# srndpty/kobato-eyes

Hardware: AMD Instinct MI355X
Metric: images/s (pHash + all-pairs Hamming scan + cluster membership) (higher is better)
Workload: dtype u8 luma, int32 taps (i8 matrix cores), f64 DCT, 1-bit Hamming products (fp4 matrix cores, exact)

## Files before the change

kobato-eyes_amd/csrc/ke_hash.hip:

```cpp
#include <cstdlib>

#include "ke_internal.h"
#include "dct_table.h"
#include "ke_hash_select.h"
#include "ke_resample_plan.h"

namespace {

constexpr int kPrecisionBits = 22;

__device__ __forceinline__ int clip8_fixed(int acc) {
    int v = acc >> kPrecisionBits;
    return v < 0 ? 0 : (v > 255 ? 255 : v);
}

__device__ __forceinline__ int luma_of(const uint8_t *p, int ch) {
    if (ch == 1) return p[0];
    return (int)((19595u * p[0] + 38470u * p[1] + 7471u * p[2] + 0x8000u) >> 16);
}

template <int AXIS>
__global__ __launch_bounds__(256) void ke_resample_pass(const uint8_t *__restrict__ src,
                                                         const uint64_t *__restrict__ offsets, uint64_t stride,
                                                         int ch, int w, int h, const int32_t *__restrict__ bounds,
// ... 159 lines not shown
    tile32_coeffs<false>(s_tile, s_T, s_cf[0], tid);
    tile32_coeffs<true>(s_tile, s_T, s_cf[1], tid);
    for (int k = wv; k < 8; k += 4) {
        const float *base = s_cf[k >> 2];
        auto coef = [&](int i) {
            const bool neg = ((k & 1) && (i & 1)) != ((k & 2) && ((i >> 3) & 1));
            return neg ? -base[i] : base[i];
        };
        float r[8];
#pragma unroll
        for (int j = 0; j < 8; ++j) r[j] = coef(1 + j);
#pragma unroll
        for (int i = 8; i < 56; i += 8)
#pragma unroll
            for (int j = 0; j < 8; ++j) r[j] = r[j] + coef(1 + i + j);
        float res = ((r[0] + r[1]) + (r[2] + r[3])) + ((r[4] + r[5]) + (r[6] + r[7]));
#pragma unroll
        for (int i = 56; i < 63; ++i) res = res + coef(1 + i);
        const float mean = res / 63.0f;
        const unsigned long long m = __ballot(coef(lane) > mean);
        if (lane == 0) turned[slot * 8 + k] = __brevll(m);
    }
}

__device__ __forceinline__ uint32_t luma4_biased(uint32_t d0, uint32_t d1, uint32_t d2) {
    constexpr uint32_t CHI = 0x001D964Cu, CLO = 0x002F468Bu, START = 0x8000u - 0x800000u;
    const uint32_t p0 = d0;
    const uint32_t p1 = __builtin_amdgcn_alignbyte(d1, d0, 3);
    const uint32_t p2 = __builtin_amdgcn_alignbyte(d2, d1, 2);
    const uint32_t s0 = (__builtin_amdgcn_udot4(p0, CHI, 0u, false) << 8) + __builtin_amdgcn_udot4(p0, CLO, START, false);
    const uint32_t s1 = (__builtin_amdgcn_udot4(p1, CHI, 0u, false) << 8) + __builtin_amdgcn_udot4(p1, CLO, START, false);
    const uint32_t s2 = (__builtin_amdgcn_udot4(p2, CHI, 0u, false) << 8) + __builtin_amdgcn_udot4(p2, CLO, START, false);
    const uint32_t s3 = (__builtin_amdgcn_udot4(d2, CHI << 8, 0u, false) << 8) + __builtin_amdgcn_udot4(d2, CLO << 8, START, false);
    const uint32_t lo = __builtin_amdgcn_perm(s1, s0, 0x0C0C0602u);
    const uint32_t hi = __builtin_amdgcn_perm(s3, s2, 0x06020C0Cu);
    return lo | hi;
}

template <int C>
__device__ __forceinline__ uint32_t luma4_generic(const uint32_t *d) {
    if (C == 3) return luma4_biased(d[0], d[1], d[2]);
    if (C == 1) return d[0] ^ 0x80808080u;
    constexpr uint32_t CHI = 0x001D964Cu, CLO = 0x002F468Bu, START = 0x8000u - 0x800000u;
    uint32_t s[4];
#pragma unroll
    for (int k = 0; k < 4; ++k)
        s[k] = (__builtin_amdgcn_udot4(d[k], CHI, 0u, false) << 8) + __builtin_amdgcn_udot4(d[k], CLO, START, false);
    return __builtin_amdgcn_perm(s[1], s[0], 0x0C0C0602u) | __builtin_amdgcn_perm(s[3], s[2], 0x06020C0Cu);
}

__device__ __forceinline__ int combine_planes(int d0, int d1, int d2, int bias) {
    return (int)((uint32_t)d0 + ((uint32_t)d1 << 8) + ((uint32_t)d2 << 16) + (uint32_t)bias);
}

struct KeFusedArgs {
    const uint8_t *pixels;
    const uint64_t *offsets;
    uint64_t stride;
    const int64_t *out_idx;
    int h;
    const int32_t *mx_frag;
    int mx_base0, mx_base1;
    const int32_t *h_bias;
    const int32_t *v_packed, *v_start, *v_bias;
    int ndwv;
    int qw, qw_inv, lp;
    int w, row_bytes;
    int lt_half;
    int lt_bytes;
    int hp;
    uint64_t *phash;
    float *margin;
    uint8_t *tile32_out;
    const int32_t *mxd_frag, *hd_bias;
    const int32_t *vd_cpacked, *vd_cstart, *vd_bias;
    int ndwcv;
    int hpd;
    int x_off;
    int bands, band_rows;
    uint8_t *hs, *hsd;
    int hs_hp, hsd_hp;
    uint64_t *dhash;
    uint8_t *tile98_out;
};

template <int C>
__device__ __forceinline__ void patch_last_quad(const uint8_t *image_last_row, int w, uint8_t *lds_row) {
    for (int x = w & ~3; x < w; ++x) lds_row[x] = (uint8_t)(luma_of(image_last_row + (size_t)x * C, C) ^ 0x80);
}

__device__ __forceinline__ void band_writeout(const uint8_t *HT, int hp, int ncols, int rows, uint8_t *dst, int dst_hp, int tid,
                                              int nthreads) {
    const int wpc = (rows + 3) / 4;
    for (int e = tid; e < ncols * wpc; e += nthreads) {
        const int col = e / wpc, k = e % wpc;
        *reinterpret_cast<uint32_t *>(dst + (size_t)col * dst_hp + 4 * k) = *reinterpret_cast<const uint32_t *>(HT + col * hp + 4 * k);
    }
}

template <int NDWD>
__device__ __forceinline__ void fused_tail(const KeFusedArgs &a, uint8_t *Lt, const uint8_t *HT, const uint8_t *HTd,
                                           const int tid, const int64_t img) {
    uint8_t *T32 = Lt;
    double *Td = reinterpret_cast<double *>(Lt + 1024);
    float *cf = reinterpret_cast<float *>(Lt + 1024 + 2048);
    {
        const int yy = tid & 31, og = tid >> 5;
        const int rotv = (yy >> 4) & 1;
        const int vst = a.v_start[yy];
        const int ndwv = a.ndwv;
        int acc[4][3];
#pragma unroll
        for (int m = 0; m < 4; ++m) acc[m][0] = acc[m][1] = acc[m][2] = 0;
        for (int j = 0; j < ndwv; j += 2) {
            const int jj = j ^ (2 * rotv);
            const int32_t *cp = a.v_packed + ((size_t)yy * ndwv + jj) * 3;
            const int c00 = cp[0], c01 = cp[1], c02 = cp[2], c10 = cp[3], c11 = cp[4], c12 = cp[5];
#pragma unroll
            for (int m = 0; m < 4; ++m) {
                const uint2 v = *reinterpret_cast<const uint2 *>(
                    __builtin_assume_aligned(HT + (size_t)(og + 8 * m) * a.hp + vst + 4 * jj, 8));
                acc[m][0] = __builtin_amdgcn_sdot4((int)v.x, c00, acc[m][0], false);
                acc[m][1] = __builtin_amdgcn_sdot4((int)v.x, c01, acc[m][1], false);
                acc[m][2] = __builtin_amdgcn_sdot4((int)v.x, c02, acc[m][2], false);
                acc[m][0] = __builtin_amdgcn_sdot4((int)v.y, c10, acc[m][0], false);
                acc[m][1] = __builtin_amdgcn_sdot4((int)v.y, c11, acc[m][1], false);
                acc[m][2] = __builtin_amdgcn_sdot4((int)v.y, c12, acc[m][2], false);
            }
        }
        const int vbias = a.v_bias[yy];
#pragma unroll
        for (int m = 0; m < 4; ++m)
            T32[yy * 32 + og + 8 * m] = (uint8_t)clip8_fixed(combine_planes(acc[m][0], acc[m][1], acc[m][2], vbias));
    }
    __syncthreads();
    if (a.tile32_out)
        reinterpret_cast<uint32_t *>(a.tile32_out + (size_t)img * 1024)[tid] = reinterpret_cast<const uint32_t *>(T32)[tid];
    const int64_t slot = a.out_idx ? a.out_idx[img] : img;
    const uint64_t hv = tile32_to_phash(T32, Td, cf, tid, (a.margin && a.phash) ? a.margin + slot : nullptr);
    if (tid == 0 && a.phash) a.phash[slot] = hv;
    if (NDWD > 0) {
        __syncthreads();
        int *part = reinterpret_cast<int *>(Lt);
        uint8_t *T98 = Lt + 1024;
        if (tid < 216) {
            const int out = tid / 3, chunk = tid % 3;
            const int yy = out / 9, oc = out % 9;
            const int vc = yy * 3 + chunk;
            const int vst = a.vd_cstart[vc];
            const int nd = a.ndwcv;
            int d0 = 0, d1 = 0, d2 = 0;
            for (int j = 0; j < nd; j += 2) {
                const int32_t *cp = a.vd_cpacked + ((size_t)vc * nd + j) * 3;
                const uint2 v = *reinterpret_cast<const uint2 *>(__builtin_assume_aligned(HTd + (size_t)oc * a.hpd + vst + 4 * j, 8));
                d0 = __builtin_amdgcn_sdot4((int)v.x, cp[0], d0, false);
                d1 = __builtin_amdgcn_sdot4((int)v.x, cp[1], d1, false);
                d2 = __builtin_amdgcn_sdot4((int)v.x, cp[2], d2, false);
                d0 = __builtin_amdgcn_sdot4((int)v.y, cp[3], d0, false);
                d1 = __builtin_amdgcn_sdot4((int)v.y, cp[4], d1, false);
                d2 = __builtin_amdgcn_sdot4((int)v.y, cp[5], d2, false);
            }
            part[tid] = combine_planes(d0, d1, d2, 0);
        }
        __syncthreads();
        if (tid < 72) {
            const int yy = tid / 9;
            const uint32_t sum = (uint32_t)part[3 * tid] + (uint32_t)part[3 * tid + 1] + (uint32_t)part[3 * tid + 2] + (uint32_t)a.vd_bias[yy];
            T98[tid] = (uint8_t)clip8_fixed((int)sum);
        }
        __syncthreads();
        if (a.tile98_out && tid < 72) a.tile98_out[(size_t)img * 72 + tid] = T98[tid];
        if (tid < 64) {
            const int r = tid >> 3, c = tid & 7;
            const unsigned long long m = __ballot(T98[r * 9 + c + 1] > T98[r * 9 + c]);
            if (tid == 0 && a.dhash) a.dhash[a.out_idx ? a.out_idx[img] : img] = __brevll(m);
        }
    }
}

int upload_dct_tables(ke_ctx *ctx) {
    if (ctx->dct_tables_ready) return KE_OK;
    KE_HIP(ctx, hipMemcpyToSymbol(HIP_SYMBOL(c_C32), KE_C32, sizeof(KE_C32)));
    KE_HIP(ctx, hipMemcpyToSymbol(HIP_SYMBOL(c_C16), KE_C16, sizeof(KE_C16)));
    KE_HIP(ctx, hipMemcpyToSymbol(HIP_SYMBOL(c_C8), KE_C8, sizeof(KE_C8)));
    ctx->dct_tables_ready = true;
    return KE_OK;
}

constexpr int kRTM = kKeTileRowsMx;
typedef int ke_v4i __attribute__((ext_vector_type(4)));

template <int W64, int KS, bool DH, bool GEN, int C, bool UNAL>
__global__ __launch_bounds__(256, 2) void ke_phash_fused_mx(const KeFusedArgs a) {
    static_assert(!UNAL || GEN, "rows that are not a multiple of 4 pixels need the run-time row length");
    constexpr uint32_t QB = 4u * C;
    constexpr int W = 64 * W64;
    constexpr int QPT = kRTM * (W / 4) / 256;
    const int QW = GEN ? a.qw : W / 4;
    const int QUADS_PER_TILE = kRTM * QW;
    const int LP = GEN ? a.lp : W + 16;
    constexpr int KD = (W64 + 1) / 2;
    extern __shared__ __attribute__((aligned(16))) uint8_t smem[];
    uint8_t *Lt = smem;
    uint8_t *HT = smem + a.lt_bytes;
    uint8_t *HTd = HT + 32 * a.hp;
    uint8_t *X = smem + a.x_off;
    const int tid = threadIdx.x;
    const int lane = tid & 63, wv = tid >> 6;
    const int64_t img = a.bands ? blockIdx.x / a.bands : blockIdx.x;
    const int y_begin = a.bands ? (int)(blockIdx.x % a.bands) * a.band_rows : 0;
    const uint32_t row_bytes = UNAL ? (uint32_t)a.row_bytes : (uint32_t)QW * QB;
    const uint8_t *src = a.pixels + (a.offsets ? a.offsets[img] : (uint64_t)img * a.stride) + (size_t)y_begin * row_bytes;
    const int h = a.bands ? min(a.band_rows, a.h - y_begin) : a.h;
    const uint32_t image_bytes = (uint32_t)(a.h - y_begin) * row_bytes;

    const int mt = wv >> 1, jt = wv & 1;
    ke_v4i bf[KS][3];
#pragma unroll
    for (int s = 0; s < KS; ++s)
#pragma unroll
        for (int p = 0; p < 3; ++p)
            bf[s][p] = reinterpret_cast<const ke_v4i *>(a.mx_frag)[((jt * KS + s) * 3 + p) * 64 + lane];
    constexpr int KDR = DH ? KD : 1;
    ke_v4i bd[KDR][3];
    int dbias = 0;
    if (DH) {
#pragma unroll
        for (int d = 0; d < KDR; ++d)
#pragma unroll
            for (int p = 0; p < 3; ++p)
                bd[d][p] = reinterpret_cast<const ke_v4i *>(a.mxd_frag)[((jt * KD + d) * 3 + p) * 64 + lane];
        dbias = a.hd_bias[(lane & 15) < 9 ? (lane & 15) : 8];
    }
    const int ocol = 16 * jt + (lane & 15);
    const int hbias = a.h_bias[ocol];
    const int a_off = (16 * mt + (lane & 15)) * LP + (jt ? a.mx_base1 : a.mx_base0) + 16 * (lane >> 4);
    const int d_off = (16 * mt + (lane & 15)) * LP + 64 * KD * jt + 16 * (lane >> 4);
    uint8_t *ht_dst = HT + (size_t)ocol * a.hp + 16 * mt + 4 * (lane >> 4);
    uint8_t *htd_dst = HTd + (size_t)(lane & 15) * a.hpd + 16 * mt + 4 * (lane >> 4);
    ke_v4i *x_slot = reinterpret_cast<ke_v4i *>(X + mt * 1024 + lane * 16);

    uint32_t raw[QPT][C];
    auto load_tile = [&](int t) {
// ... 46 lines not shown
        }
        if (DH) {
            const uint8_t *dp = cur + d_off;
#pragma unroll
            for (int d = 0; d < KDR; ++d) {
                const ke_v4i av = *reinterpret_cast<const ke_v4i *>(__builtin_assume_aligned(dp + 64 * d, 16));
#pragma unroll
                for (int p = 0; p < 3; ++p) dacc[p] = __builtin_amdgcn_mfma_i32_16x16x64_i8(av, bd[d][p], dacc[p], 0, 0, 0);
            }
        }
        *reinterpret_cast<uint32_t *>(ht_dst + t * kRTM) = pack_rows(acc[0], acc[1], acc[2], hbias);
        ke_v4i part;
#pragma unroll
        for (int i = 0; i < 4; ++i) part[i] = combine_planes(dacc[0][i], dacc[1][i], dacc[2][i], 0);
        return part;
    };
    ke_v4i carry = {0, 0, 0, 0};
    auto finish_dhash = [&](int t) {
        const ke_v4i other = x_slot[(t & 1) * 128];
        const ke_v4i zero = {0, 0, 0, 0};
        const ke_v4i sum = carry + other;
        const uint32_t packed = pack_rows(sum, zero, zero, dbias);
        if ((lane & 15) < 9) *reinterpret_cast<uint32_t *>(htd_dst + t * kRTM) = packed;
    };
    auto hpass = [&](int t, const uint8_t *cur) {
        if (!DH) {
            products(t, cur);
        } else if (jt) {
            x_slot[(t & 1) * 128] = products(t, cur);
        } else {
            if (t > 0) finish_dhash(t - 1);
            carry = products(t, cur);
        }
    };

    const int ntiles = (h + kRTM - 1) / kRTM;
    load_tile(0);
    store_luma(Lt);
    __syncthreads();
    for (int t = 0; t + 1 < ntiles; ++t) {
        load_tile(t + 1);
        __builtin_amdgcn_sched_barrier(0);
        hpass(t, Lt + (t & 1) * a.lt_half);
        __builtin_amdgcn_sched_barrier(0);
        store_luma(Lt + ((t + 1) & 1) * a.lt_half);
        __syncthreads();
    }
    if (UNAL) {
        if (tid == 0 && y_begin + h == a.h)
            patch_last_quad<C>(src + (size_t)(h - 1) * row_bytes, a.w, Lt + ((ntiles - 1) & 1) * a.lt_half + ((h - 1) - (ntiles - 1) * kRTM) * LP);
        __syncthreads();
    }
    hpass(ntiles - 1, Lt + ((ntiles - 1) & 1) * a.lt_half);
    __syncthreads();
    if (DH) {
        if (!jt) finish_dhash(ntiles - 1);
        __syncthreads();
    }
    if (a.bands) {
        band_writeout(HT, a.hp, 32, h, a.hs + (size_t)img * 32 * a.hs_hp + y_begin, a.hs_hp, tid, 256);
        if (DH) band_writeout(HTd, a.hpd, 9, h, a.hsd + (size_t)img * 9 * a.hsd_hp + y_begin, a.hsd_hp, tid, 256);
        return;
    }
    fused_tail<(DH ? 1 : 0)>(a, Lt, HT, HTd, tid, img);
}

constexpr int kRTW = kKeTileRowsWide;

template <int KSH, int QPT, bool DH, int KDW, int C, bool UNAL>
__global__ __launch_bounds__(512, 1) void ke_phash_fused_wide(const KeFusedArgs a) {
    constexpr uint32_t QB = 4u * C;
    extern __shared__ __attribute__((aligned(16))) uint8_t smem[];
    uint8_t *Lt = smem;
    uint8_t *HT = smem + a.lt_bytes;
    uint8_t *HTd = HT + 32 * a.hp;
    uint8_t *X = smem + a.x_off;
    const int tid = threadIdx.x;
    const int lane = tid & 63, wv = tid >> 6;
    const int jt = wv & 1, kh = wv >> 1;
    const int64_t img = a.bands ? blockIdx.x / a.bands : blockIdx.x;
    const int y_begin = a.bands ? (int)(blockIdx.x % a.bands) * a.band_rows : 0;
    const int QW = a.qw, LP = a.lp;
    const uint32_t row_bytes = UNAL ? (uint32_t)a.row_bytes : (uint32_t)QW * QB;
    const uint8_t *src = a.pixels + (a.offsets ? a.offsets[img] : (uint64_t)img * a.stride) + (size_t)y_begin * row_bytes;
    const int h = a.bands ? min(a.band_rows, a.h - y_begin) : a.h;
    const int quads_per_tile = kRTW * QW;
    const uint32_t image_bytes = (uint32_t)(a.h - y_begin) * row_bytes;

    ke_v4i bf[KSH][3];
#pragma unroll
    for (int s = 0; s < KSH; ++s)
#pragma unroll
        for (int p = 0; p < 3; ++p)
            bf[s][p] = reinterpret_cast<const ke_v4i *>(a.mx_frag)[((jt * 4 * KSH + kh * KSH + s) * 3 + p) * 64 + lane];
    const int ocol = 16 * jt + (lane & 15);
    const int hbias = a.h_bias[ocol];
    const int a_off = (lane & 15) * LP + (jt ? a.mx_base1 : a.mx_base0) + 64 * KSH * kh + 16 * (lane >> 4);
    uint8_t *ht_dst = HT + (size_t)ocol * a.hp + 4 * (lane >> 4);
    ke_v4i *x_slot = reinterpret_cast<ke_v4i *>(X) + jt * 192 + lane;
    constexpr int KDR = DH ? KDW : 1;
    ke_v4i bd[KDR][3];
    int dbias = 0;
    if (DH) {
#pragma unroll
        for (int d = 0; d < KDR; ++d)
#pragma unroll
            for (int p = 0; p < 3; ++p)
                bd[d][p] = reinterpret_cast<const ke_v4i *>(a.mxd_frag)[((wv * KDW + d) * 3 + p) * 64 + lane];
        dbias = a.hd_bias[(lane & 15) < 9 ? (lane & 15) : 8];
    }
    const int d_off = (lane & 15) * LP + 64 * KDW * wv + 16 * (lane >> 4);
    uint8_t *htd_dst = HTd + (size_t)(lane & 15) * a.hpd + 4 * (lane >> 4);
    ke_v4i *xd_slot = reinterpret_cast<ke_v4i *>(X) + 768 + lane;

    uint32_t raw[QPT][C];
    auto load_tile = [&](int t) {
        const uint32_t tile_off = UNAL ? (uint32_t)t * (kRTW * row_bytes) : (uint32_t)t * ((uint32_t)quads_per_tile * QB);
// ... 58 lines not shown
    auto dfinish = [&](int t) {
        const ke_v4i *xs = xd_slot + (t & 1) * 448;
        ke_v4i sum = dcarry;
#pragma unroll
        for (int k = 0; k < 7; ++k) sum += xs[64 * k];
        uint32_t packed = 0;
#pragma unroll
        for (int i = 0; i < 4; ++i) packed |= (uint32_t)clip8_fixed((int)((uint32_t)sum[i] + (uint32_t)dbias)) << (8 * i);
        if ((lane & 15) < 9) *reinterpret_cast<uint32_t *>(htd_dst + t * kRTW) = packed ^ 0x80808080u;
    };
    auto finish = [&](int t) {
        const ke_v4i *xs = x_slot + (t & 1) * 384;
        const ke_v4i sum = carry + xs[0] + xs[64] + xs[128];
        uint32_t packed = 0;
#pragma unroll
        for (int i = 0; i < 4; ++i) packed |= (uint32_t)clip8_fixed((int)((uint32_t)sum[i] + (uint32_t)hbias)) << (8 * i);
        *reinterpret_cast<uint32_t *>(ht_dst + t * kRTW) = packed ^ 0x80808080u;
    };
    auto hpass = [&](int t, const uint8_t *cur) {
        if (kh) {
            x_slot[(t & 1) * 384 + (kh - 1) * 64] = products(cur);
        } else {
            if (t > 0) finish(t - 1);
            carry = products(cur);
        }
        if (DH) {
            if (wv) {
                xd_slot[(t & 1) * 448 + (wv - 1) * 64] = dproducts(cur);
            } else {
                if (t > 0) dfinish(t - 1);
                dcarry = dproducts(cur);
            }
        }
    };

    const int ntiles = (h + kRTW - 1) / kRTW;
    load_tile(0);
    store_luma(Lt);
    __syncthreads();
    for (int t = 0; t + 1 < ntiles; ++t) {
        load_tile(t + 1);
        __builtin_amdgcn_sched_barrier(0);
        hpass(t, Lt + (t & 1) * a.lt_half);
        __builtin_amdgcn_sched_barrier(0);
        store_luma(Lt + ((t + 1) & 1) * a.lt_half);
        __syncthreads();
    }
    if (UNAL) {
        if (tid == 0 && y_begin + h == a.h)
            patch_last_quad<C>(src + (size_t)(h - 1) * row_bytes, a.w, Lt + ((ntiles - 1) & 1) * a.lt_half + ((h - 1) - (ntiles - 1) * kRTW) * LP);
        __syncthreads();
    }
    hpass(ntiles - 1, Lt + ((ntiles - 1) & 1) * a.lt_half);
    __syncthreads();
    if (!kh) finish(ntiles - 1);
    if (DH && !wv) dfinish(ntiles - 1);
    __syncthreads();
    if (a.bands) {
        band_writeout(HT, a.hp, 32, h, a.hs + (size_t)img * 32 * a.hs_hp + y_begin, a.hs_hp, tid, 512);
        if (DH) band_writeout(HTd, a.hpd, 9, h, a.hsd + (size_t)img * 9 * a.hsd_hp + y_begin, a.hsd_hp, tid, 512);
        return;
    }
    if (tid >= 256) return;
    fused_tail<(DH ? 1 : 0)>(a, Lt, HT, HTd, tid, img);
}

struct KeBandArgs {
    const uint8_t *pixels;
    const uint64_t *offsets;
    uint64_t stride;
    int w, h;
    int qr;
    int lp;
    int rt;
    int band_rows;
    int bands;
    int nout;
    int nout_total;
    int out_first;
    int cpo_log2;
    int vcp_log2;
    const int32_t *cpacked, *cstart, *cxor, *bias;
    int lt_half;
    int bp;
    uint8_t *hs;
    int hp;
};

template <int NDWC, int C, bool ALIGNED>
__global__ __launch_bounds__(256, 3) void ke_hband(const KeBandArgs a) {
    constexpr int QPT = 8;
    constexpr int DW = C;
    extern __shared__ __attribute__((aligned(16))) uint8_t smem[];
    const int tid = threadIdx.x;
    const int64_t img = blockIdx.x / a.bands;
    const int band = blockIdx.x % a.bands;
    const uint8_t *src = a.pixels + (a.offsets ? a.offsets[img] : (uint64_t)img * a.stride);
    const int y_begin = band * a.band_rows;
    const int y_end = min(a.h, y_begin + a.band_rows);
    const uintptr_t last_dword = ((uintptr_t)src + (uintptr_t)a.w * a.h * C - 1) & ~(uintptr_t)3;

    const int vcl = tid & ((1 << a.vcp_log2) - 1);
    const int rg = tid >> a.vcp_log2, RG = 256 >> a.vcp_log2;
    const int nvc = a.nout << a.cpo_log2;
    const int vloc = vcl < nvc ? vcl : nvc - 1;
    const int o = vloc >> a.cpo_log2;
    const int vc = vloc + (a.out_first << a.cpo_log2);
    const bool writer = vcl < nvc && (vloc & ((1 << a.cpo_log2) - 1)) == 0;
    const int xs = a.cxor[vc];
    int ck[NDWC][3];
#pragma unroll
    for (int p = 0; p < NDWC / 2; ++p)
#pragma unroll
        for (int e = 0; e < 2; ++e)
#pragma unroll
            for (int c = 0; c < 3; ++c) ck[2 * p + e][c] = a.cpacked[((size_t)vc * NDWC + 2 * (p ^ xs) + e) * 3 + c];
    const int cst = a.cstart[vc];
// ... 462 lines not shown
    return launch_vtile(ctx, a.hs, a.hp, g.n, ow, oh, ax.vt, d_tiles, sw);
}

int resample_generic(ke_ctx *ctx, const KeHashGroup &g, int ow, int oh, uint8_t *d_tiles, int filter, const float *box, KeRanPlan *ran) {
    KeAxes ax;
    KE_TRY(fetch_axes(ctx, g, ow, oh, filter, box, &ax));
    const KeAxisCoeffs *chz = ax.hz, *cvt = ax.vt;
    const KeGenericPlan p = ke_plan_generic(g.w, g.h, ow, oh);
    if (ran) { ran->banded = false; ran->generic = p; }
    for (int64_t f = 0; f < g.n; f += p.max_n) {
        const KeHashGroup s = ke_sub_group(g, f, std::min(p.max_n, g.n - f));
        uint8_t *dst = d_tiles + (size_t)f * ow * oh;
        void *tmp;
        KE_TRY(ke_reserve(ctx, KE_BUF_TMP, (size_t)s.n * p.mid_bytes, &tmp));
        if (!ke_fits_one_launch(s.n * p.b0)) return declined(ctx, KE_DECLINE_ONE_LAUNCH);
        if (!p.vertical_first) {
            hipLaunchKernelGGL(ke_resample_pass<0>, dim3((unsigned)(s.n * p.b0)), dim3(256), 0, ctx->stream, s.pixels, s.offsets,
                               s.stride, s.channels, s.w, s.h, chz->d_bounds, chz->d_kk, chz->ksize, ow, (uint8_t *)tmp, p.b0);
            hipLaunchKernelGGL(ke_resample_pass<1>, dim3((unsigned)(s.n * p.b1)), dim3(256), 0, ctx->stream, (const uint8_t *)tmp,
                               (const uint64_t *)nullptr, (uint64_t)p.mid_bytes, 1, p.mid_w, p.mid_h, cvt->d_bounds, cvt->d_kk,
                               cvt->ksize, oh, dst, p.b1);
        } else {
            hipLaunchKernelGGL(ke_resample_pass<1>, dim3((unsigned)(s.n * p.b0)), dim3(256), 0, ctx->stream, s.pixels, s.offsets,
                               s.stride, s.channels, s.w, s.h, cvt->d_bounds, cvt->d_kk, cvt->ksize, oh, (uint8_t *)tmp, p.b0);
            hipLaunchKernelGGL(ke_resample_pass<0>, dim3((unsigned)(s.n * p.b1)), dim3(256), 0, ctx->stream, (const uint8_t *)tmp,
                               (const uint64_t *)nullptr, (uint64_t)p.mid_bytes, 1, p.mid_w, p.mid_h, chz->d_bounds, chz->d_kk,
                               chz->ksize, ow, dst, p.b1);
        }
        KE_HIP(ctx, hipGetLastError());
    }
    return KE_OK;
}

int resample_to_tiles(ke_ctx *ctx, const KeHashGroup &g, int ow, int oh, uint8_t *d_tiles, const KeHashSwitches &sw, bool try_strips,
                      int filter = KE_FILTER_LANCZOS, const float *box = nullptr, KeRanPlan *ran = nullptr) {
    int rc = try_strips ? resample_strips(ctx, g, ow, oh, d_tiles, sw) : KE_EUNSUPPORTED;
    if (rc == KE_EUNSUPPORTED) rc = resample_banded(ctx, g, ow, oh, d_tiles, sw, filter, box, ran);
    if (rc == KE_EUNSUPPORTED) rc = resample_generic(ctx, g, ow, oh, d_tiles, filter, box, ran);
    return rc;
}

using KeFusedKernel = void (*)(KeFusedArgs);
#define KE_SP_KERNEL(F, A0, A1, A2, A3, A4, A5, LO, HI) ke_phash_fused_##F<A0, A1, A2, A3, A4, A5>,
const KeFusedKernel kSpKernels[] = {KE_SINGLE_PASS_ROWS(KE_SP_KERNEL)};
#undef KE_SP_KERNEL
static_assert(sizeof(kSpKernels) / sizeof(kSpKernels[0]) == kKeSpRowCount, "one kernel per row");

struct KeBandTarget {
    const KeSpBandPlan *plan;
    uint8_t *hs, *hsd;
};

int launch_fused(ke_ctx *ctx, int r, const KeHashGroup &g, const KeAxisCoeffs *ch, const KeAxisCoeffs *cv, uint64_t *d_phash,
                 uint8_t *d_tile32, uint64_t *d_dhash, uint8_t *d_tile98, const KeBandTarget *bands) {
    const bool DH = kKeSpRows[r].dh();
    const KeFusedSteps steps = ke_plan_fused_steps(r, g.w);
    if (steps.why) return declined(ctx, steps.why);
    const KeMxTable *mx = ke_get_mx(ctx, ch, steps.ks);
    if (!mx) return ke_fail(ctx, KE_EHIP, "coefficient upload failed");
    const KeAxisCoeffs *chd = nullptr, *cvd = nullptr;
    const KeMxTable *mxd = nullptr;
    const KeChunkTable *tv = nullptr;
    if (DH) {
        chd = ke_get_coeffs(ctx, g.w, 9); cvd = ke_get_coeffs(ctx, g.h, 8);
        if (!chd || !cvd) return ke_fail(ctx, KE_EHIP, "coefficient upload failed");
        mxd = ke_get_mx(ctx, chd, steps.ksd); tv = ke_get_chunks(ctx, cvd, 3);
        if (!mxd || !tv) return ke_fail(ctx, KE_EHIP, "coefficient upload failed");
    }
    const KeFusedPlan p = ke_plan_fused(r, g.w, g.h, g.n, steps, *mx, cv->span, mxd, tv, bands ? bands->plan : nullptr);
    if (p.why) return declined(ctx, p.why);
    KeFusedArgs a;
    std::memset(&a, 0, sizeof a);
    a.pixels = g.pixels; a.offsets = g.offsets; a.stride = g.stride; a.out_idx = g.out_idx; a.h = g.h;
    a.h_bias = ch->d_bias;
    a.v_packed = cv->d_packed; a.v_start = cv->d_start; a.v_bias = cv->d_bias;
    a.ndwv = cv->ndw;
    a.mx_frag = mx->d_frag; a.mx_base0 = mx->base[0]; a.mx_base1 = mx->base[1];
    if (bands) { a.bands = bands->plan->bands; a.band_rows = bands->plan->band_rows; a.hs = bands->hs; a.hsd = bands->hsd; a.hs_hp = bands->plan->hs_hp; a.hsd_hp = bands->plan->hsd_hp; }
    a.qw = p.qw; a.qw_inv = p.qw_inv; a.lp = p.lp;
    a.w = g.w; a.row_bytes = p.row_bytes;
    a.lt_half = p.lt_half; a.lt_bytes = 2 * p.lt_half;
    a.hp = p.hp; a.hpd = p.hpd; a.x_off = p.x_off;
    a.phash = d_phash; a.tile32_out = d_tile32; a.margin = ctx->margin_cur;
    if (DH) {
        a.mxd_frag = mxd->d_frag;
        a.hd_bias = chd->d_bias;
        a.vd_cpacked = tv->d_cpacked; a.vd_cstart = tv->d_cstart; a.vd_bias = cvd->d_bias;
        a.ndwcv = tv->ndwc;
        a.dhash = d_dhash; a.tile98_out = d_tile98;
    }
    if (p.raise_lds_limit)
        KE_HIP(ctx, hipFuncSetAttribute(reinterpret_cast<const void *>(kSpKernels[r]), hipFuncAttributeMaxDynamicSharedMemorySize, (int)p.lds));
    hipLaunchKernelGGL(kSpKernels[r], dim3((unsigned)p.workgroups), dim3(p.threads), p.lds, ctx->stream, a);
    KE_HIP(ctx, hipGetLastError());
    return KE_OK;
}

int dispatch_single_pass(ke_ctx *ctx, const KeHashGroup &g, bool want_d, uint64_t *d_phash, uint8_t *d_t32, uint64_t *d_dhash,
                         uint8_t *d_t98, const KeBandTarget *bands, bool *did_d) {
    *did_d = false;
    const KeSpShape shape{g.w, g.h, g.channels, g.misaligned, (uintptr_t)g.pixels % 4 == 0, g.offsets || g.stride % 4 == 0,
                          want_d, bands != nullptr};
    int rows[kKeSpMaxCandidates];
    const int n = ke_single_pass_candidates(shape, rows);
    if (!n) return KE_EUNSUPPORTED;
    const KeAxisCoeffs *ch = ke_get_coeffs(ctx, g.w, 32);
    const KeAxisCoeffs *cv = ke_get_coeffs(ctx, g.h, 32);
    if (!ch || !cv) return ke_fail(ctx, KE_EHIP, "coefficient upload failed");
    for (int k = 0; k < n; ++k) {
        const bool dh = kKeSpRows[rows[k]].dh();
        const int rc = launch_fused(ctx, rows[k], g, ch, cv, d_phash, d_t32, dh ? d_dhash : nullptr, dh ? d_t98 : nullptr, bands);
        if (rc != KE_EUNSUPPORTED) { *did_d = dh && rc == KE_OK; return rc; }
    }
    return KE_EUNSUPPORTED;
}

int resample_single_pass_banded(ke_ctx *ctx, const KeHashGroup &g, uint8_t *d_t32, uint8_t *d_t98, const KeHashSwitches &sw, bool *did_d) {
    *did_d = false;
    const KeAxisCoeffs *cvt = ke_get_coeffs(ctx, g.h, 32);
    const KeAxisCoeffs *cvd = d_t98 ? ke_get_coeffs(ctx, g.h, 8) : nullptr;
    if (!cvt || (d_t98 && !cvd)) return ke_fail(ctx, KE_EHIP, "coefficient upload failed");
    const KeSpBandPlan p = ke_plan_sp_bands(shape_of(g), d_t98 != nullptr, cvt->span, cvd ? cvd->span : 0, ctx->cu_count);
    if (p.why) return declined(ctx, p.why);
    void *hs;
    KE_TRY(ke_reserve(ctx, KE_BUF_TMP, p.scratch_bytes, &hs));
    const KeBandTarget bands{&p, (uint8_t *)hs, cvd ? (uint8_t *)hs + (size_t)g.n * 32 * p.hs_hp : nullptr};
    KE_TRY(dispatch_single_pass(ctx, g, d_t98 != nullptr, nullptr, nullptr, nullptr, nullptr, &bands, did_d));
    KE_TRY(launch_vtile(ctx, bands.hs, p.hs_hp, g.n, 32, 32, cvt, d_t32, sw));
    if (*did_d) KE_TRY(launch_vtile(ctx, bands.hsd, p.hsd_hp, g.n, 9, 8, cvd, d_t98, sw));
    return KE_OK;
}

}

int ke_launch_hash_group(ke_ctx *ctx, const KeHashGroup &g, uint64_t *d_phash, uint64_t *d_dhash, uint8_t *d_tile32_out,
                         uint8_t *d_tile98_out, hipStream_t fused_stream) {
    KE_TRY(upload_dct_tables(ctx));
    const KeHashSwitches sw = read_switches();
    const bool want_p = d_phash || d_tile32_out, want_d = d_dhash || d_tile98_out;
    bool p_done = false, d_done = false;
    if (want_p && g.n >= ke_fused_min_images((int64_t)g.w * g.h * g.channels, sw)) {
        bool did_d = false;
        hipStream_t home = ctx->stream;
        if (fused_stream) ctx->stream = fused_stream;
        const int rc = dispatch_single_pass(ctx, g, want_d, d_phash, d_tile32_out, d_dhash, d_tile98_out, nullptr, &did_d);
        ctx->stream = home;
        if (rc == KE_OK) { p_done = true; d_done = did_d; }
        else if (rc != KE_EUNSUPPORTED) return rc;
    }
    if ((want_p && !p_done) || (want_d && !d_done)) {
        const int64_t chunk = ke_chunk_images(ke_hash_scratch_per_image(g.h));
        for (int64_t f = 0; f < g.n; f += chunk) {
            const KeHashGroup s = ke_sub_group(g, f, std::min(chunk, g.n - f));
            const int64_t slot0 = g.out_idx ? 0 : f;
            void *t32 = nullptr, *t98 = nullptr;
            bool d_here = false;
            if (want_d && !d_done) {
                if (d_tile98_out) t98 = d_tile98_out + (size_t)f * 72;
                else KE_TRY(ke_reserve(ctx, KE_BUF_TILE98, (size_t)s.n * 72, &t98));
            }
            if (want_p && !p_done) {
                if (d_tile32_out) t32 = d_tile32_out + (size_t)f * 1024;
                else KE_TRY(ke_reserve(ctx, KE_BUF_TILE32, (size_t)s.n * 1024, &t32));
                int rb = resample_single_pass_banded(ctx, s, (uint8_t *)t32, (uint8_t *)t98, sw, &d_here);
                if (rb == KE_EUNSUPPORTED) rb = resample_to_tiles(ctx, s, 32, 32, (uint8_t *)t32, sw, true);
                KE_TRY(rb);
            }
            if (want_d && !d_done && !d_here) KE_TRY(resample_to_tiles(ctx, s, 9, 8, (uint8_t *)t98, sw, true));
            uint64_t *ph = (d_phash && !p_done) ? d_phash + slot0 : nullptr;
            uint64_t *dh = (d_dhash && !d_done) ? d_dhash + slot0 : nullptr;
            if (ph || dh) {
                hipLaunchKernelGGL(ke_tiles_to_hashes, dim3((unsigned)s.n), dim3(256), 0, ctx->stream, (const uint8_t *)t32,
                                   (const uint8_t *)t98, s.out_idx, ph, dh, (ph && ctx->margin_cur) ? ctx->margin_cur + slot0 : nullptr);
                KE_HIP(ctx, hipGetLastError());
            }
        }
    }
    return KE_OK;
}

int ke_launch_tiles_turned(ke_ctx *ctx, const uint8_t *d_tile32, const int64_t *d_out_idx, int64_t n, uint64_t *d_turned) {
    if (n <= 0) return KE_OK;
    if (!ke_fits_one_launch(n)) return ke_fail(ctx, KE_EUNSUPPORTED, "too many tiles for one launch");
    KE_TRY(upload_dct_tables(ctx));
    hipLaunchKernelGGL(ke_tiles_to_phash_turned, dim3((unsigned)n), dim3(256), 0, ctx->stream, d_tile32, d_out_idx, d_turned);
    KE_HIP(ctx, hipGetLastError());
    return KE_OK;
}

int ke_launch_resize_group(ke_ctx *ctx, const KeHashGroup &g, int ow, int oh, int filter, uint8_t *d_tiles, const float *box) {
    if (ow <= 0 || oh <= 0 || ow > 4096 || oh > 4096) return ke_fail(ctx, KE_EINVAL, "bad output size %dx%d", ow, oh);
    const KeHashSwitches sw = read_switches();
    const int64_t chunk = ke_chunk_images(ke_resize_scratch_per_image(ow, oh, g.h));
    for (int64_t f = 0; f < g.n; f += chunk) {
        KeRanPlan ran;
        KE_TRY(resample_to_tiles(ctx, ke_sub_group(g, f, std::min(chunk, g.n - f)), ow, oh, d_tiles + (size_t)f * ow * oh, sw, false, filter, box, &ran));
        int32_t *rp = ctx->resize_plan;
        for (int k = 0; k < KE_RP_COUNT; ++k) rp[k] = -1;
// ... 77 lines not shown
```

kobato-eyes_amd/csrc/ke_resample_plan.h:

```cpp
#pragma once
#include <algorithm>
#include <cstddef>
#include <cstdint>

#include "ke_coeffs.h"
#include "ke_hash_select.h"

struct KeHashSwitches {
    bool fused_min_set = false;
    int64_t fused_min_images = 0;
    bool vtile_valu = false;
};

struct KePlanShape {
    int w, h, channels;
    int64_t n;
    bool misaligned, base_dword, stride_dword, has_offsets;
};

enum KeDecline {
    KE_PLAN_OK = 0,
    KE_DECLINE_ONE_LAUNCH,
    KE_DECLINE_HB_VERTICAL_FIRST,
    KE_DECLINE_HB_SHAPE,
// ... 194 lines not shown

struct KeSpBandPlan {
    KeDecline why;
    int bands, band_rows;
    int hs_hp, hsd_hp;
    size_t scratch_bytes;
};

inline KeSpBandPlan ke_plan_sp_bands(const KePlanShape &g, bool want_d, int vspan, int vdspan, int cu_count) {
    KeSpBandPlan p{};
    if (ke_taller_than_100_widths(g.w, g.h) || g.h < 16) { p.why = KE_DECLINE_SPB_SHAPE; return p; }
    const int64_t fill = (4 * (int64_t)cu_count + g.n - 1) / g.n;
    const bool both = want_d && g.channels == 3;
    const int64_t fixed = (g.w <= 768 && !(both && g.w > 512)) ? 64 * (int64_t)(g.w + 32) + (both ? 4096 : 0)
                                                               : 32 * (int64_t)(g.w + 32) + 12288 + (both ? 14336 : 0);
    int64_t max_rows = (80 * 1024 - fixed) / (both ? 41 : 32) / 32 * 32 - 32;
    if (max_rows < 128) max_rows = 1024;
    max_rows = std::min<int64_t>(max_rows, 1024);
    const int64_t bands = std::max<int64_t>((g.h + max_rows - 1) / max_rows, std::min<int64_t>(fill, (g.h + 63) / 64));
    p.band_rows = (int)(((g.h + bands - 1) / bands + 31) / 32 * 32);
    p.bands = (g.h + p.band_rows - 1) / p.band_rows;
    p.hs_hp = ke_column_pitch(vspan, g.h);
    p.hsd_hp = want_d ? ke_column_pitch(vdspan, g.h) : 8;
    p.scratch_bytes = (size_t)g.n * (32 * (size_t)p.hs_hp + (want_d ? 9 * (size_t)p.hsd_hp : 0)) + 8192;
    return p;
}

constexpr int kKeTileRowsMx = 32, kKeTileRowsWide = 16;

struct KeFusedSteps {
    KeDecline why;
    int ks;
    int ksd;
};

inline KeFusedSteps ke_plan_fused_steps(int r, int W) {
    const KeSpRow &row = kKeSpRows[r];
    const bool wide = row.family == KE_SP_WIDE;
    KeFusedSteps s{KE_PLAN_OK, wide ? 4 * row.t[0] : row.t[1], wide ? 8 * row.t[3] : 2 * ((row.t[0] + 1) / 2)};
    if ((W % 4 != 0) != row.unal() || (wide ? kKeTileRowsWide * ((W + 3) / 4) > 512 * row.t[1] : W < row.w_lo || W > row.w_hi)) s.why = KE_DECLINE_FU_WIDTH;
    return s;
}

struct KeFusedPlan {
    KeDecline why;
    int qw, qw_inv, lp, lt_half, hp, hpd, x_off;
    int row_bytes;
    int threads;
    int64_t workgroups;
    size_t lds;
    bool raise_lds_limit;
};

inline KeFusedPlan ke_plan_fused(int r, int W, int h, int64_t n, const KeFusedSteps &s, const KeMxTable &mx, int vspan, const KeMxTable *mxd,
                                 const KeChunkTable *vd, const KeSpBandPlan *bands) {
    const KeSpRow &row = kKeSpRows[r];
    const bool wide = row.family == KE_SP_WIDE, DH = row.dh();
    const int C = row.channels();
    const int rt = wide ? kKeTileRowsWide : kKeTileRowsMx;
    const bool exact = !wide && !row.t[3];
    KeFusedPlan p{};
    p.threads = wide ? 512 : 256;
    if (mx.tiles != 2 || mx.ks != s.ks) { p.why = KE_DECLINE_FU_TABLE; return p; }
    const int rows_padded = bands ? bands->band_rows : ((h + rt - 1) / rt) * rt;
    const int overhang = std::max(0, std::max(std::max(mx.base[0], mx.base[1]) + 64 * s.ks, DH ? 64 * s.ksd : 0) - W);
    p.qw = (W + 3) / 4;
    p.row_bytes = W * C;
    p.qw_inv = (int)(uint32_t)((0x100000000ull + (uint64_t)p.qw - 1) / (uint64_t)p.qw);
    p.lp = exact ? W + 16 : (((W + 15) / 16 + 1) | 1) * 16;
    p.lt_half = (rt * p.lp + overhang + 15) & ~15;
    p.hp = ((std::max(bands ? 0 : vspan, rows_padded) + 7) & ~7) + 8;
    p.hpd = 8;
    p.lds = (size_t)2 * p.lt_half + (size_t)32 * p.hp;
    if (!wide) p.lds = std::max<size_t>(p.lds, 4096);
    if (DH) {
        if (mxd->tiles != 1 || mxd->base[0] != 0 || mxd->ks != s.ksd) { p.why = KE_DECLINE_FU_DH_TABLE; return p; }
        p.hpd = ((std::max(bands ? 0 : vd->cspan, rows_padded) + 7) & ~7) + 8;
        p.lds += (size_t)9 * p.hpd;
    }
    if (wide || DH) {
        p.lds = (p.lds + 15) & ~(size_t)15;
        p.x_off = (int)p.lds;
        p.lds += wide ? 2 * 2 * 3 * 1024 + (DH ? 2 * 7 * 1024 : 0) : 4096;
    }
    if (p.lds > 150 * 1024) { p.why = KE_DECLINE_FU_LDS; return p; }
    if (!bands && p.lds > 80 * 1024 && p.lds - (size_t)(32 * (p.hp - 136)) - (DH ? (size_t)(9 * (p.hpd - 136)) : 0) <= 80 * 1024) { p.why = KE_DECLINE_FU_BANDS_FIT; return p; }
    p.raise_lds_limit = p.lds > 64 * 1024;
    p.workgroups = n * (bands ? bands->bands : 1);
    if (!ke_fits_one_launch(p.workgroups)) p.why = KE_DECLINE_ONE_LAUNCH;
    return p;
}

struct KeGenericPlan {
    bool vertical_first;
    int mid_w, mid_h;
    size_t mid_bytes;
    int64_t max_n;
    int b0, b1;
};

inline KeGenericPlan ke_plan_generic(int w, int h, int ow, int oh) {
    KeGenericPlan p;
    p.vertical_first = ke_taller_than_100_widths(w, h) && oh < h;
    p.mid_w = p.vertical_first ? w : ow;
    p.mid_h = p.vertical_first ? oh : h;
    p.mid_bytes = (size_t)p.mid_w * p.mid_h;
    p.max_n = ke_chunk_images(p.mid_bytes);
    p.b0 = (int)((p.mid_bytes + 255) / 256);
    p.b1 = (ow * oh + 255) / 256;
    return p;
}
```

Measured before the change: 8.755 million.

## Run fused kernel vertical-pass tail on i8 MFMA with early fragment prefetch

```diff
diff --git a/kobato-eyes_amd/csrc/ke_hash.hip b/kobato-eyes_amd/csrc/ke_hash.hip
--- a/kobato-eyes_amd/csrc/ke_hash.hip
+++ b/kobato-eyes_amd/csrc/ke_hash.hip
@@ -235,6 +235,8 @@
 __device__ __forceinline__ int combine_planes(int d0, int d1, int d2, int bias) {
     return (int)((uint32_t)d0 + ((uint32_t)d1 << 8) + ((uint32_t)d2 << 16) + (uint32_t)bias);
 }
+
+typedef int ke_v4i __attribute__((ext_vector_type(4)));
 
 struct KeFusedArgs {
     const uint8_t *pixels;
@@ -265,6 +267,10 @@
     int hs_hp, hsd_hp;
     uint64_t *dhash;
     uint8_t *tile98_out;
+    const int32_t *vmx_frag;
+    int vmx_ks, vmx_base0, vmx_base1;
+    const int32_t *vdmx_frag;
+    int vdmx_kq;
 };
 
 template <int C>
@@ -361,6 +367,130 @@
     }
 }
 
+template <int N>
+__device__ __forceinline__ void tail_load(ke_v4i (&fa)[N][3], const ke_v4i *fr, int s) {
+#pragma unroll
+    for (int i = 0; i < N; ++i)
+#pragma unroll
+        for (int p = 0; p < 3; ++p) fa[i][p] = fr[((s + i) * 3 + p) * 64];
+}
+template <int N>
+__device__ __forceinline__ void tail_mac(ke_v4i (&acc)[3], const ke_v4i (&fa)[N][3], const uint8_t *bp, int s) {
+#pragma unroll
+    for (int i = 0; i < N; ++i) {
+        const ke_v4i bv = *reinterpret_cast<const ke_v4i *>(__builtin_assume_aligned(bp + 64 * (s + i), 16));
+#pragma unroll
+        for (int p = 0; p < 3; ++p) acc[p] = __builtin_amdgcn_mfma_i32_16x16x64_i8(fa[i][p], bv, acc[p], 0, 0, 0);
+    }
+}
+
+
+struct KeTailRegs {
+    ke_v4i fa[6][3], da[2][3], vbias;
+    int dbias;
+};
+
+struct KeTailLane {
+    int lane, wv, mt, nt;
+    __device__ __forceinline__ explicit KeTailLane(int tid) {
+        asm volatile("" : "+v"(tid));
+        lane = tid & 63; wv = __builtin_amdgcn_readfirstlane(tid >> 6); mt = wv >> 1; nt = wv & 1;
+    }
+};
+
+constexpr bool ke_tail_prefetch_early(bool dh, int dead) { return dead >= (dh ? 124 : 100); }
+
+template <bool DH, int G>
+__device__ __forceinline__ void tail_prefetch(const KeFusedArgs &a, const int tid, KeTailRegs &r) {
+    const KeTailLane l(tid);
+    const int ks = a.vmx_ks;
+    const ke_v4i *fr = reinterpret_cast<const ke_v4i *>(a.vmx_frag) + (size_t)l.mt * ks * 3 * 64 + l.lane;
+    if (DH) {
+        tail_load<2>(r.da, reinterpret_cast<const ke_v4i *>(a.vdmx_frag) + (size_t)l.wv * a.vdmx_kq * 3 * 64 + l.lane, 0);
+        r.dbias = a.vd_bias[min(tid / 9, 7)];
+    }
+    r.vbias = *reinterpret_cast<const ke_v4i *>(a.v_bias + 16 * l.mt + 4 * (l.lane >> 4));
+    if (G == 6 && ks >= 6) {
+        tail_load<6>(r.fa, fr, 0);
+    } else {
+        tail_load<3>(reinterpret_cast<ke_v4i (&)[3][3]>(r.fa), fr, 0);
+    }
+}
+
+template <bool DH, int G>
+__device__ __forceinline__ void fused_tail_mx(const KeFusedArgs &a, const KeTailRegs &r, uint8_t *Lt, uint8_t *HT, const uint8_t *HTd,
+                                              uint8_t *X, const int tid, const int64_t img) {
+    uint8_t *T32 = Lt;
+    double *Td = reinterpret_cast<double *>(Lt + 1024);
+    float *cf = reinterpret_cast<float *>(Lt + 1024 + 2048);
+    uint8_t *T98 = HT;
+    const KeTailLane l(tid);
+    const int lane = l.lane, wv = l.wv, mt = l.mt, nt = l.nt;
+    const int ks = a.vmx_ks, kq = DH ? a.vdmx_kq : 0;
+    const ke_v4i *fr = reinterpret_cast<const ke_v4i *>(a.vmx_frag) + (size_t)mt * ks * 3 * 64 + lane;
+    const ke_v4i *dfr = DH ? reinterpret_cast<const ke_v4i *>(a.vdmx_frag) + (size_t)wv * kq * 3 * 64 + lane : nullptr;
+    const uint8_t *bp = HT + (size_t)(16 * nt + (lane & 15)) * a.hp + (mt ? a.vmx_base1 : a.vmx_base0) + 16 * (lane >> 4);
+    const uint8_t *dbp = HTd + (size_t)min(lane & 15, 8) * a.hpd + 64 * wv * kq + 16 * (lane >> 4);
+    const ke_v4i vbias = r.vbias;
+    ke_v4i acc[3], dacc[3];
+#pragma unroll
+    for (int p = 0; p < 3; ++p) acc[p] = dacc[p] = ke_v4i{0, 0, 0, 0};
+    int s;
+    if (G == 6 && ks >= 6) {
+        tail_mac<6>(acc, r.fa, bp, 0);
+        s = 6;
+    } else {
+        tail_mac<3>(acc, reinterpret_cast<const ke_v4i (&)[3][3]>(r.fa), bp, 0);
+        s = 3;
+    }
+    for (; s < ks; s += 3) {
+        ke_v4i fa[3][3];
+        tail_load<3>(fa, fr, s);
+        tail_mac<3>(acc, fa, bp, s);
+    }
+#pragma unroll
+    for (int i = 0; i < 4; ++i)
+        T32[(16 * mt + 4 * (lane >> 4) + i) * 32 + 16 * nt + (lane & 15)] = (uint8_t)clip8_fixed(combine_planes(acc[0][i], acc[1][i], acc[2][i], vbias[i]));
+    if (DH) {
+        tail_mac<2>(dacc, r.da, dbp, 0);
+        for (int d = 2; d < kq; d += 2) {
+            ke_v4i fa[2][3];
+            tail_load<2>(fa, dfr, d);
+            tail_mac<2>(dacc, fa, dbp, d);
+        }
+        ke_v4i part;
+#pragma unroll
+        for (int i = 0; i < 4; ++i) part[i] = combine_planes(dacc[0][i], dacc[1][i], dacc[2][i], 0);
+        reinterpret_cast<ke_v4i *>(X)[wv * 64 + lane] = part;
+    }
+    __syncthreads();
+    if (a.tile32_out)
+        reinterpret_cast<uint32_t *>(a.tile32_out + (size_t)img * 1024)[tid] = reinterpret_cast<const uint32_t *>(T32)[tid];
+    if (DH && tid < 72) {
+        const int yy = tid / 9, oc = tid % 9;
+        const int *xp = reinterpret_cast<const int *>(X) + (16 * (yy >> 2) + oc) * 4 + (yy & 3);
+        const uint32_t sum = (uint32_t)xp[0] + (uint32_t)xp[256] + (uint32_t)xp[512] + (uint32_t)xp[768] + (uint32_t)r.dbias;
+        T98[tid] = (uint8_t)clip8_fixed((int)sum);
+    }
+    const int64_t slot = a.out_idx ? a.out_idx[img] : img;
+    const uint64_t hv = tile32_to_phash(T32, Td, cf, tid, (a.margin && a.phash) ? a.margin + slot : nullptr);
+    if (tid == 0 && a.phash) a.phash[slot] = hv;
+    if (DH) {
+        if (a.tile98_out && tid < 72) a.tile98_out[(size_t)img * 72 + tid] = T98[tid];
+        if (tid < 64) {
+            const int r = tid >> 3, c = tid & 7;
+            const unsigned long long m = __ballot(T98[r * 9 + c + 1] > T98[r * 9 + c]);
+            if (tid == 0 && a.dhash) a.dhash[slot] = __brevll(m);
+        }
+    }
+}
+
+__device__ __forceinline__ const KeFusedArgs &tail_args() {
+    auto kp = __builtin_amdgcn_kernarg_segment_ptr();
+    asm volatile("" : "+s"(kp));
+    return *(const KeFusedArgs *)kp;
+}
+
 int upload_dct_tables(ke_ctx *ctx) {
     if (ctx->dct_tables_ready) return KE_OK;
     KE_HIP(ctx, hipMemcpyToSymbol(HIP_SYMBOL(c_C32), KE_C32, sizeof(KE_C32)));
@@ -371,7 +501,6 @@
 }
 
 constexpr int kRTM = kKeTileRowsMx;
-typedef int ke_v4i __attribute__((ext_vector_type(4)));
 
 template <int W64, int KS, bool DH, bool GEN, int C, bool UNAL>
 __global__ __launch_bounds__(256, 2) void ke_phash_fused_mx(const KeFusedArgs a) {
@@ -524,6 +653,11 @@
         __syncthreads();
     }
     hpass(ntiles - 1, Lt + ((ntiles - 1) & 1) * a.lt_half);
+    const KeFusedArgs &ta = tail_args();
+    const bool tail_mx = ta.vmx_frag != nullptr;
+    KeTailRegs tr;
+    constexpr bool EARLY = ke_tail_prefetch_early(DH, 12 * KS + (DH ? 12 * KD : 0) + QPT * C);
+    if (EARLY && tail_mx) tail_prefetch<DH, EARLY ? 6 : 3>(ta, tid, tr);
     __syncthreads();
     if (DH) {
         if (!jt) finish_dhash(ntiles - 1);
@@ -534,7 +668,10 @@
         if (DH) band_writeout(HTd, a.hpd, 9, h, a.hsd + (size_t)img * 9 * a.hsd_hp + y_begin, a.hsd_hp, tid, 256);
         return;
     }
-    fused_tail<(DH ? 1 : 0)>(a, Lt, HT, HTd, tid, img);
+    if (tail_mx) {
+        if (!EARLY) tail_prefetch<DH, EARLY ? 6 : 3>(ta, tid, tr);
+        fused_tail_mx<DH, EARLY ? 6 : 3>(ta, tr, Lt, HT, HTd, X, tid, img);
+    } else fused_tail<(DH ? 1 : 0)>(a, Lt, HT, HTd, tid, img);
 }
 
 constexpr int kRTW = kKeTileRowsWide;
@@ -699,6 +836,11 @@
         __syncthreads();
     }
     hpass(ntiles - 1, Lt + ((ntiles - 1) & 1) * a.lt_half);
+    const KeFusedArgs &ta = tail_args();
+    const bool tail_mx = ta.vmx_frag != nullptr;
+    KeTailRegs tr;
+    constexpr bool EARLY = ke_tail_prefetch_early(DH, 12 * KSH + (DH ? 12 * KDW : 0) + QPT * C);
+    if (EARLY && tail_mx && tid < 256) tail_prefetch<DH, EARLY ? 6 : 3>(ta, tid, tr);
     __syncthreads();
     if (!kh) finish(ntiles - 1);
     if (DH && !wv) dfinish(ntiles - 1);
@@ -709,7 +851,10 @@
         return;
     }
     if (tid >= 256) return;
-    fused_tail<(DH ? 1 : 0)>(a, Lt, HT, HTd, tid, img);
+    if (tail_mx) {
+        if (!EARLY) tail_prefetch<DH, EARLY ? 6 : 3>(ta, tid, tr);
+        fused_tail_mx<DH, EARLY ? 6 : 3>(ta, tr, Lt, HT, HTd, X, tid, img);
+    } else fused_tail<(DH ? 1 : 0)>(a, Lt, HT, HTd, tid, img);
 }
 
 struct KeBandArgs {
@@ -1278,7 +1423,7 @@
 };
 
 int launch_fused(ke_ctx *ctx, int r, const KeHashGroup &g, const KeAxisCoeffs *ch, const KeAxisCoeffs *cv, uint64_t *d_phash,
-                 uint8_t *d_tile32, uint64_t *d_dhash, uint8_t *d_tile98, const KeBandTarget *bands) {
+                 uint8_t *d_tile32, uint64_t *d_dhash, uint8_t *d_tile98, const KeBandTarget *bands, const KeHashSwitches &sw) {
     const bool DH = kKeSpRows[r].dh();
     const KeFusedSteps steps = ke_plan_fused_steps(r, g.w);
     if (steps.why) return declined(ctx, steps.why);
@@ -1295,6 +1440,17 @@
     }
     const KeFusedPlan p = ke_plan_fused(r, g.w, g.h, g.n, steps, *mx, cv->span, mxd, tv, bands ? bands->plan : nullptr);
     if (p.why) return declined(ctx, p.why);
+    KeFusedTailPlan tail{false, p.hp, p.hpd, p.x_off, p.lds, p.raise_lds_limit, 0, 0};
+    const KeMxTable *vmx = nullptr, *vdmx = nullptr;
+    if (!bands && !sw.vtile_valu) {
+        const KeMxTable *nat = ke_get_mx(ctx, cv), *natd = DH ? ke_get_mx(ctx, cvd) : nullptr;
+        if (!nat || (DH && !natd)) return ke_fail(ctx, KE_EHIP, "coefficient upload failed");
+        const int want = ke_fused_tail_steps(nat->ks), wantd = DH ? ke_fused_tail_dsteps(natd->ks) : 0;
+        vmx = want == nat->ks ? nat : ke_get_mx(ctx, cv, want);
+        if (DH) vdmx = wantd == natd->ks ? natd : ke_get_mx(ctx, cvd, wantd);
+        if (!vmx || (DH && !vdmx)) return ke_fail(ctx, KE_EHIP, "coefficient upload failed");
+        tail = ke_plan_fused_tail(r, p, *vmx, vdmx, sw);
+    }
     KeFusedArgs a;
     std::memset(&a, 0, sizeof a);
     a.pixels = g.pixels; a.offsets = g.offsets; a.stride = g.stride; a.out_idx = g.out_idx; a.h = g.h;
@@ -1306,7 +1462,7 @@
     a.qw = p.qw; a.qw_inv = p.qw_inv; a.lp = p.lp;
     a.w = g.w; a.row_bytes = p.row_bytes;
     a.lt_half = p.lt_half; a.lt_bytes = 2 * p.lt_half;
-    a.hp = p.hp; a.hpd = p.hpd; a.x_off = p.x_off;
+    a.hp = tail.hp; a.hpd = tail.hpd; a.x_off = tail.x_off;
     a.phash = d_phash; a.tile32_out = d_tile32; a.margin = ctx->margin_cur;
     if (DH) {
         a.mxd_frag = mxd->d_frag;
@@ -1315,15 +1471,19 @@
         a.ndwcv = tv->ndwc;
         a.dhash = d_dhash; a.tile98_out = d_tile98;
     }
-    if (p.raise_lds_limit)
-        KE_HIP(ctx, hipFuncSetAttribute(reinterpret_cast<const void *>(kSpKernels[r]), hipFuncAttributeMaxDynamicSharedMemorySize, (int)p.lds));
-    hipLaunchKernelGGL(kSpKernels[r], dim3((unsigned)p.workgroups), dim3(p.threads), p.lds, ctx->stream, a);
+    if (tail.on_mx) {
+        a.vmx_frag = vmx->d_frag; a.vmx_ks = tail.ks; a.vmx_base0 = vmx->base[0]; a.vmx_base1 = vmx->base[1];
+        if (DH) { a.vdmx_frag = vdmx->d_frag; a.vdmx_kq = tail.kdq; }
+    }
+    if (tail.raise_lds_limit)
+        KE_HIP(ctx, hipFuncSetAttribute(reinterpret_cast<const void *>(kSpKernels[r]), hipFuncAttributeMaxDynamicSharedMemorySize, (int)tail.lds));
+    hipLaunchKernelGGL(kSpKernels[r], dim3((unsigned)p.workgroups), dim3(p.threads), tail.lds, ctx->stream, a);
     KE_HIP(ctx, hipGetLastError());
     return KE_OK;
 }
 
 int dispatch_single_pass(ke_ctx *ctx, const KeHashGroup &g, bool want_d, uint64_t *d_phash, uint8_t *d_t32, uint64_t *d_dhash,
-                         uint8_t *d_t98, const KeBandTarget *bands, bool *did_d) {
+                         uint8_t *d_t98, const KeBandTarget *bands, const KeHashSwitches &sw, bool *did_d) {
     *did_d = false;
     const KeSpShape shape{g.w, g.h, g.channels, g.misaligned, (uintptr_t)g.pixels % 4 == 0, g.offsets || g.stride % 4 == 0,
                           want_d, bands != nullptr};
@@ -1335,7 +1495,7 @@
     if (!ch || !cv) return ke_fail(ctx, KE_EHIP, "coefficient upload failed");
     for (int k = 0; k < n; ++k) {
         const bool dh = kKeSpRows[rows[k]].dh();
-        const int rc = launch_fused(ctx, rows[k], g, ch, cv, d_phash, d_t32, dh ? d_dhash : nullptr, dh ? d_t98 : nullptr, bands);
+        const int rc = launch_fused(ctx, rows[k], g, ch, cv, d_phash, d_t32, dh ? d_dhash : nullptr, dh ? d_t98 : nullptr, bands, sw);
         if (rc != KE_EUNSUPPORTED) { *did_d = dh && rc == KE_OK; return rc; }
     }
     return KE_EUNSUPPORTED;
@@ -1351,7 +1511,7 @@
     void *hs;
     KE_TRY(ke_reserve(ctx, KE_BUF_TMP, p.scratch_bytes, &hs));
     const KeBandTarget bands{&p, (uint8_t *)hs, cvd ? (uint8_t *)hs + (size_t)g.n * 32 * p.hs_hp : nullptr};
-    KE_TRY(dispatch_single_pass(ctx, g, d_t98 != nullptr, nullptr, nullptr, nullptr, nullptr, &bands, did_d));
+    KE_TRY(dispatch_single_pass(ctx, g, d_t98 != nullptr, nullptr, nullptr, nullptr, nullptr, &bands, sw, did_d));
     KE_TRY(launch_vtile(ctx, bands.hs, p.hs_hp, g.n, 32, 32, cvt, d_t32, sw));
     if (*did_d) KE_TRY(launch_vtile(ctx, bands.hsd, p.hsd_hp, g.n, 9, 8, cvd, d_t98, sw));
     return KE_OK;
@@ -1369,7 +1529,7 @@
         bool did_d = false;
         hipStream_t home = ctx->stream;
         if (fused_stream) ctx->stream = fused_stream;
-        const int rc = dispatch_single_pass(ctx, g, want_d, d_phash, d_tile32_out, d_dhash, d_tile98_out, nullptr, &did_d);
+        const int rc = dispatch_single_pass(ctx, g, want_d, d_phash, d_tile32_out, d_dhash, d_tile98_out, nullptr, sw, &did_d);
         ctx->stream = home;
         if (rc == KE_OK) { p_done = true; d_done = did_d; }
         else if (rc != KE_EUNSUPPORTED) return rc;
diff --git a/kobato-eyes_amd/csrc/ke_resample_plan.h b/kobato-eyes_amd/csrc/ke_resample_plan.h
--- a/kobato-eyes_amd/csrc/ke_resample_plan.h
+++ b/kobato-eyes_amd/csrc/ke_resample_plan.h
@@ -270,6 +270,19 @@
     bool raise_lds_limit;
 };
 
+inline size_t ke_fused_lds(bool wide, bool DH, int lt_half, int hp, int hpd, int *x_off) {
+    size_t lds = (size_t)2 * lt_half + (size_t)32 * hp;
+    if (!wide) lds = std::max<size_t>(lds, 4096);
+    if (DH) lds += (size_t)9 * hpd;
+    *x_off = 0;
+    if (wide || DH) {
+        lds = (lds + 15) & ~(size_t)15;
+        *x_off = (int)lds;
+        lds += wide ? 2 * 2 * 3 * 1024 + (DH ? 2 * 7 * 1024 : 0) : 4096;
+    }
+    return lds;
+}
+
 inline KeFusedPlan ke_plan_fused(int r, int W, int h, int64_t n, const KeFusedSteps &s, const KeMxTable &mx, int vspan, const KeMxTable *mxd,
                                  const KeChunkTable *vd, const KeSpBandPlan *bands) {
     const KeSpRow &row = kKeSpRows[r];
@@ -289,24 +302,47 @@
     p.lt_half = (rt * p.lp + overhang + 15) & ~15;
     p.hp = ((std::max(bands ? 0 : vspan, rows_padded) + 7) & ~7) + 8;
     p.hpd = 8;
-    p.lds = (size_t)2 * p.lt_half + (size_t)32 * p.hp;
-    if (!wide) p.lds = std::max<size_t>(p.lds, 4096);
     if (DH) {
         if (mxd->tiles != 1 || mxd->base[0] != 0 || mxd->ks != s.ksd) { p.why = KE_DECLINE_FU_DH_TABLE; return p; }
         p.hpd = ((std::max(bands ? 0 : vd->cspan, rows_padded) + 7) & ~7) + 8;
-        p.lds += (size_t)9 * p.hpd;
-    }
-    if (wide || DH) {
-        p.lds = (p.lds + 15) & ~(size_t)15;
-        p.x_off = (int)p.lds;
-        p.lds += wide ? 2 * 2 * 3 * 1024 + (DH ? 2 * 7 * 1024 : 0) : 4096;
-    }
+    }
+    p.lds = ke_fused_lds(wide, DH, p.lt_half, p.hp, p.hpd, &p.x_off);
     if (p.lds > 150 * 1024) { p.why = KE_DECLINE_FU_LDS; return p; }
     if (!bands && p.lds > 80 * 1024 && p.lds - (size_t)(32 * (p.hp - 136)) - (DH ? (size_t)(9 * (p.hpd - 136)) : 0) <= 80 * 1024) { p.why = KE_DECLINE_FU_BANDS_FIT; return p; }
     p.raise_lds_limit = p.lds > 64 * 1024;
     p.workgroups = n * (bands ? bands->bands : 1);
     if (!ke_fits_one_launch(p.workgroups)) p.why = KE_DECLINE_ONE_LAUNCH;
     return p;
+}
+
+constexpr int kKeTailStepGroup = 3, kKeTailDStepGroup = 2;
+inline int ke_fused_tail_steps(int natural_ks) { return (natural_ks + kKeTailStepGroup - 1) / kKeTailStepGroup * kKeTailStepGroup; }
+inline int ke_fused_tail_dsteps(int natural_ks) {
+    const int per_wave = ((natural_ks + 3) / 4 + kKeTailDStepGroup - 1) / kKeTailDStepGroup * kKeTailDStepGroup;
+    return 4 * per_wave;
+}
+
+struct KeFusedTailPlan {
+    bool on_mx;
+    int hp, hpd, x_off;
+    size_t lds;
+    bool raise_lds_limit;
+    int ks, kdq;
+};
+
+inline KeFusedTailPlan ke_plan_fused_tail(int r, const KeFusedPlan &p, const KeMxTable &vmx, const KeMxTable *vdmx, const KeHashSwitches &sw) {
+    const KeSpRow &row = kKeSpRows[r];
+    const bool wide = row.family == KE_SP_WIDE, DH = row.dh();
+    KeFusedTailPlan t{false, p.hp, p.hpd, p.x_off, p.lds, p.raise_lds_limit, 0, 0};
+    if (sw.vtile_valu || vmx.tiles != 2 || vmx.ks % kKeTailStepGroup) return t;
+    if (DH && (!vdmx || vdmx->tiles != 1 || vdmx->base[0] != 0 || vdmx->ks % (4 * kKeTailDStepGroup))) return t;
+    auto odd16 = [](int bytes) { return (((bytes + 15) / 16) | 1) * 16; };
+    const int hp = odd16(std::max(p.hp, std::max(vmx.base[0], vmx.base[1]) + 64 * vmx.ks));
+    const int hpd = DH ? odd16(std::max(p.hpd, 64 * vdmx->ks)) : p.hpd;
+    int x_off = 0;
+    const size_t lds = ke_fused_lds(wide, DH, p.lt_half, hp, hpd, &x_off);
+    if (lds > 150 * 1024 || (p.lds <= 80 * 1024 && lds > 80 * 1024)) return t;
+    return {true, hp, hpd, x_off, lds, lds > 64 * 1024, vmx.ks, DH ? vdmx->ks / 4 : 0};
 }
 
 struct KeGenericPlan {
```

After: 9.033 million, median of 6. 3.2% higher.
